# coop-columb/two-tower-amazon-recommender

Hardware: AMD Instinct MI355X
Metric: user-item pairs/sec (train step) + embedding-gather HBM GB/s, 1/2/4/8 MI355X (higher is better)
Workload: dtype f32; 1 GPU; cfg3: 5000000 users x 10000000 items, emb_dim 128, towers 128->256->128, batch 8192, in-batch sampled softmax T=0.1, sgd lr 1e-3, ids U; global_batch=8192, parallelism=single GPU

## Files before the change

### two_tower_amazon_recommender_amd/csrc/score.hip

```cpp
#include "common.h"

namespace {

using tt::f32x4;
using tt::f32x16;
typedef __bf16 bf16x4 __attribute__((ext_vector_type(4)));
typedef __bf16 bf16x8 __attribute__((ext_vector_type(8)));
typedef short s16x4 __attribute__((ext_vector_type(4)));

constexpr float kLog2e = 1.44269504088896340736f;
constexpr float kLn2 = 0.69314718055994530942f;
constexpr float kNegBig = -1.0e30f;

enum { MODE_FWD = 0, MODE_BWD = 1, MODE_FUSED = 2, MODE_RANK = 3, MODE_FUSED_S = 4, MODE_BWD_S = 5 };
constexpr float kRescaleThr = 8.0f;

struct ScoreArgs {
  const float* R;
  const float* K;
  int64_t n_r, n_c;
  int64_t diag;
  float c1;
  const float* a_r;
  const float* s_r;
  const float* a_c;
  const float* s_c;
  const int64_t* id_r;
  const int64_t* id_c;
  int nsplit;
  int64_t c_per_split;
  float* part_m;
  float* part_l;
  float* pos2;
  float* slab;
  const float* h_r;
  const float* h_c;
  const int64_t* pos_idx;
  int32_t* part_cnt;
  float* S;
  int64_t ldS;
};

template <int D, int PREC>
struct Geo {
  static constexpr int LS = D + 4;
  static constexpr int NG = D / 8;
  static constexpr int NB = D / 32;
  static constexpr int KS = D / 16;
  static constexpr int HALF_B = 32 * 256;
  static constexpr int PIECE_B = (D / 128) * HALF_B;
  static constexpr int TILE_F = PREC == 0 ? 32 * LS : 3 * PIECE_B / 4;
  static constexpr int BUF_F = TILE_F + 160;
  static constexpr int LDS_BYTES = 2 * BUF_F * 4;
};

struct Bf3 {
  __bf16 hi, mid, lo;
};
__device__ __forceinline__ Bf3 split3(float x) {
  Bf3 o;
  o.hi = (__bf16)x;
  const float r1 = x - (float)o.hi;
  o.mid = (__bf16)r1;
  o.lo = (__bf16)(r1 - (float)o.mid);
  return o;
}

__device__ __forceinline__ int img_off(int row, int ch) { return 256 * row + 16 * (ch ^ (((row & 3) << 2) | ((row >> 2) & 3))); }

constexpr int kBwdSWaves = 2;
constexpr int kSPrefetch = 2;
#ifndef TT_LOOP_LAMBDA
#define TT_LOOP_LAMBDA 0
#endif
constexpr int kTilesPerBarrier = 2;
constexpr int kTilesPerBarrierBwdS = kTilesPerBarrier;
template <int D, int MODE, int PREC>
constexpr int tiles_per_barrier() {
  if (PREC == 0 && D <= 128 && MODE == MODE_BWD_S) return kTilesPerBarrierBwdS;
  return (PREC == 0 && D <= 128 && (MODE == MODE_BWD || MODE == MODE_FUSED || MODE == MODE_FUSED_S))
             ? kTilesPerBarrier : 1;
}

template <int D, int MODE, int PREC>
constexpr bool split_d() {
  return PREC == 1 && D == 256 && (MODE == MODE_BWD || MODE == MODE_FUSED || MODE == MODE_FUSED_S);
}
template <int D, int MODE, bool HAS_IDS, bool HAS_HN, int PREC>
constexpr int rf_lds_groups() {
  if (PREC == 0 && D == 256 && (MODE == MODE_FUSED || MODE == MODE_FUSED_S) && (HAS_IDS || HAS_HN))
    return (HAS_IDS && HAS_HN) ? 10 : (HAS_HN ? 8 : 5);
  if (PREC == 0 && D == 128 && MODE == MODE_BWD && HAS_IDS && HAS_HN) return 2;
  return 0;
}
template <int D, int MODE, int PREC, int WAVES>
constexpr int rows_per_wg() { return (split_d<D, MODE, PREC>() ? WAVES / 2 : WAVES) * 32; }

template <int D, int MODE, bool HAS_IDS, bool HAS_HN, int WAVES, int PREC>
__global__ __launch_bounds__(WAVES * 64, (WAVES == 8 ? 2 : (D <= 128 ? ((MODE == MODE_BWD_S && PREC == 0) ? kBwdSWaves : 2) : 1))) void score_kernel(ScoreArgs p) {
  constexpr bool IS_FUSED = MODE == MODE_FUSED || MODE == MODE_FUSED_S;
  constexpr bool IS_BWD = MODE == MODE_BWD || MODE == MODE_BWD_S;
  constexpr bool FROM_S = MODE == MODE_BWD_S, TO_S = MODE == MODE_FUSED_S;
  using G_ = Geo<D, PREC>;
  constexpr int LS = G_::LS, NG = G_::NG, NB = G_::NB, TILE_F = G_::TILE_F, BUF_F = G_::BUF_F;
  constexpr int HALF_B = G_::HALF_B, PIECE_B = G_::PIECE_B;
  constexpr bool SPLIT = split_d<D, MODE, PREC>();
  constexpr int KS = SPLIT ? G_::KS / 2 : G_::KS;
  constexpr int NBW = SPLIT ? NB / 2 : NB;
  static_assert(PREC == 0 || D % 128 == 0, "bf16x3: dim 128 / 256 only (whole [32][128] bf16 images)");
  constexpr int ROW4 = D / 4;
  constexpr int THREADS = WAVES * 64;
  constexpr int NV = (32 * ROW4 + THREADS - 1) / THREADS;
  extern __shared__ __attribute__((aligned(16))) float smem[];

  const int tid = threadIdx.x;
  const int lane = tid & 63;
  const int wave = tid >> 6;
  const int h = lane >> 5;
  const int ln = lane & 31;

  const int split = __builtin_amdgcn_readfirstlane((int)(blockIdx.x % (unsigned)p.nsplit));
  const int64_t rblk = __builtin_amdgcn_readfirstlane((int)(blockIdx.x / (unsigned)p.nsplit));
  const int hw = SPLIT ? (wave & 1) : 0;
  const int64_t r0w = rblk * rows_per_wg<D, MODE, PREC, WAVES>() + (SPLIT ? wave >> 1 : wave) * 32;
  const int64_t r = r0w + ln;
  const bool r_ok = r < p.n_r;
  const int64_t c_begin = (int64_t)split * p.c_per_split;
  int64_t c_end = c_begin + p.c_per_split;
  if (c_end > p.n_c) c_end = p.n_c;
  const int ntiles = __builtin_amdgcn_readfirstlane(c_end > c_begin ? (int)((c_end - c_begin + 31) >> 5) : 0);

  constexpr bool RLO_LDS = PREC == 1 && WAVES == 8;
  constexpr int TPB = tiles_per_barrier<D, MODE, PREC>();
  static_assert(!(SPLIT && RLO_LDS), "wave-pair exchange buffer and the LDS lo fragments share one LDS region");
  static_assert(!SPLIT || TPB == 1, "the wave-pair exchange relies on one workgroup barrier per tile");
  constexpr int NBUF = 2 * TPB;
  constexpr int RFL = rf_lds_groups<D, MODE, HAS_IDS, HAS_HN, PREC>();
  constexpr int RFR = PREC == 0 ? NG - RFL : 1;
  f32x4 rf[RFR];
  f32x4* rfl = reinterpret_cast<f32x4*>(smem + NBUF * BUF_F) + (wave * (RFL > 0 ? RFL : 1)) * 64 + lane;
  bf16x8 rp[PREC == 0 ? 1 : (RLO_LDS ? 2 : 3)][PREC == 0 ? 1 : KS];
  bf16x8* rlo = reinterpret_cast<bf16x8*>(smem + NBUF * BUF_F) + (wave * KS) * 64 + lane;
  if constexpr (FROM_S) {
  } else if constexpr (PREC == 0) {
    const f32x4* R4 = reinterpret_cast<const f32x4*>(p.R + (r_ok ? r : 0) * D) + h;
#pragma unroll
    for (int g = 0; g < NG; ++g) {
      const f32x4 v = r_ok ? R4[2 * g] : f32x4{0.f, 0.f, 0.f, 0.f};
      if constexpr (RFL > 0) {
        if (g >= RFR) rfl[(g - RFR) * 64] = v; else rf[g < RFR ? g : 0] = v;
      } else {
        rf[g] = v;
      }
    }
  } else {
    const f32x4* R4 = reinterpret_cast<const f32x4*>(p.R + (r_ok ? r : 0) * D) + 2 * h + 32 * hw;
    const float live = r_ok ? 1.f : 0.f;
#pragma unroll
    for (int ks = 0; ks < KS; ++ks) {
      const f32x4 x0 = R4[4 * ks] * live;
      const f32x4 x1 = R4[4 * ks + 1] * live;
      bf16x8 lo8;
#pragma unroll
      for (int j = 0; j < 4; ++j) {
        const Bf3 u = split3(x0[j]), v = split3(x1[j]);
        rp[0][ks][j] = u.hi; rp[1][ks][j] = u.mid; lo8[j] = u.lo;
        rp[0][ks][4 + j] = v.hi; rp[1][ks][4 + j] = v.mid; lo8[4 + j] = v.lo;
      }
      if constexpr (RLO_LDS) rlo[ks * 64] = lo8;
      else rp[2][ks] = lo8;
    }
  }
  const float ar = ((IS_BWD || MODE == MODE_RANK) && p.a_r != nullptr && r_ok) ? p.a_r[r] : 0.f;
  const float sr = (IS_BWD && p.s_r != nullptr && r_ok) ? p.s_r[r] : 1.f;
  int64_t idr = 0;
  if constexpr (HAS_IDS) idr = r_ok ? p.id_r[r] : (int64_t)-1;
  const int64_t cpos = p.pos_idx != nullptr ? (r_ok ? p.pos_idx[r] : (int64_t)-1) : r + p.diag;

  f32x4 st[NV];
  float st_a = 0.f, st_s = 0.f, st_h = -3.0e38f;
  constexpr bool hn = HAS_HN;
  const float hr = (HAS_HN && p.h_r != nullptr && r_ok) ? p.h_r[r] : -3.0e38f;
  int64_t st_id = -2;
  constexpr int RPJ = THREADS / ROW4 > 0 ? THREADS / ROW4 : 1;
  const int st_row = tid / ROW4, st_col4 = tid % ROW4;
  const f32x4* kp = reinterpret_cast<const f32x4*>(p.K) + c_begin * ROW4;
  const bool has_ac = p.a_c != nullptr, has_sc = p.s_c != nullptr, has_hc = HAS_HN && p.h_c != nullptr;
  const float* acp = (has_ac ? p.a_c : p.K) + c_begin;
  const float* scp = (has_sc ? p.s_c : p.K) + c_begin;
  const float* hcp = (has_hc ? p.h_c : p.K) + c_begin;
  const int64_t* idp = nullptr;
  if constexpr (HAS_IDS) idp = p.id_c + c_begin;
  const int ncols = (int)(c_end - c_begin);

  auto load_tile = [&](int t) {
    const int nvalid = ncols - 32 * t;
    const int last = (nvalid < 32 ? nvalid : 32) - 1;
    const f32x4* src = kp + (int64_t)t * (32 * ROW4);
#pragma unroll
    for (int j = 0; j < NV; ++j) {
      const int row = st_row + j * RPJ;
      st[j] = src[(row < last ? row : last) * ROW4 + st_col4];
    }
    const int c = 32 * t + (tid < last ? tid : last);
    st_a = acp[c];
    if constexpr (HAS_HN) st_h = hcp[c];
    if constexpr (IS_BWD) st_s = scp[c];
    if constexpr (HAS_IDS) st_id = idp[c];
  };
  constexpr bool ST_FULL = NV * THREADS == 32 * ROW4;
  auto store_tile = [&](int t, int buf) {
    float* T = smem + buf * BUF_F;
    const int nvalid = ncols - 32 * t;
#pragma unroll
    for (int j = 0; j < NV; ++j) st[j] = (st_row + j * RPJ < nvalid) ? st[j] : f32x4{0.f, 0.f, 0.f, 0.f};
    if constexpr (!ST_FULL) {
#pragma unroll
      for (int j = 0; j < NV; ++j) asm volatile("" : : "v"(st[j]));
    }
    if constexpr (PREC == 0) {
      float* dst = T + st_row * LS + st_col4 * 4;
#pragma unroll
      for (int j = 0; j < NV; ++j)
        if (ST_FULL || st_row + j * RPJ < 32) *reinterpret_cast<f32x4*>(dst + j * RPJ * LS) = st[j];
    } else {
      char* img = reinterpret_cast<char*>(T);
      const int d0 = 4 * st_col4;
      const int sub = (d0 >> 7) * HALF_B + 8 * ((d0 >> 2) & 1), ch = (d0 & 127) >> 3;
#pragma unroll
      for (int j = 0; j < NV; ++j) {
        const int row = st_row + j * RPJ;
        if (ST_FULL || row < 32) {
          bf16x4 q0, q1, q2;
#pragma unroll
          for (int e = 0; e < 4; ++e) {
            const Bf3 u = split3(st[j][e]);
            q0[e] = u.hi; q1[e] = u.mid; q2[e] = u.lo;
          }
          char* dst = img + sub + img_off(row, ch);
          *reinterpret_cast<bf16x4*>(dst) = q0;
          *reinterpret_cast<bf16x4*>(dst + PIECE_B) = q1;
          *reinterpret_cast<bf16x4*>(dst + 2 * PIECE_B) = q2;
        }
      }
    }
    asm volatile("" : : "v"(st_a));
    if constexpr (IS_BWD) asm volatile("" : : "v"(st_s));
    if constexpr (HAS_HN) asm volatile("" : : "v"(st_h));
    if constexpr (HAS_IDS) asm volatile("" : : "v"(st_id));
    if (tid < 32) {
      const bool ok = tid < nvalid;
      T[TILE_F + tid] = ok ? (has_ac ? st_a : 0.f) : kNegBig;
      T[TILE_F + 32 + tid] = ok ? ((IS_BWD && has_sc) ? st_s : 1.f) : 0.f;
      if constexpr (HAS_HN) T[TILE_F + 128 + tid] = (ok && has_hc) ? st_h : -3.0e38f;
      if constexpr (HAS_IDS) reinterpret_cast<int64_t*>(T + TILE_F + 64)[tid] = ok ? st_id : (int64_t)-2;
    }
  };

  const bool frag_ok = __builtin_amdgcn_readfirstlane((int)(r0w < p.n_r)) != 0;
  auto store_S = [&](int t, const f32x16& X) {
    if (!frag_ok) return;
    const int64_t ctile = (c_begin >> 5) + t;
    float* blk = p.S + (ctile * p.ldS + (r0w >> 5)) * 1024 + ln * 32 + 4 * h;
#pragma unroll
    for (int g = 0; g < 4; ++g)
      if (!SPLIT || (g >> 1) == hw)
        *reinterpret_cast<f32x4*>(blk + 8 * g) = f32x4{X[4 * g], X[4 * g + 1], X[4 * g + 2], X[4 * g + 3]};
  };
  float* xch = smem + NBUF * BUF_F;
  auto exchange = [&](f32x16& X) {
    f32x4* mine = reinterpret_cast<f32x4*>(xch + wave * 1024) + lane;
    const f32x4* other = reinterpret_cast<const f32x4*>(xch + (wave ^ 1) * 1024) + lane;
#pragma unroll
    for (int g = 0; g < 4; ++g) mine[64 * g] = f32x4{X[4 * g], X[4 * g + 1], X[4 * g + 2], X[4 * g + 3]};
    __syncthreads();
#pragma unroll
    for (int g = 0; g < 4; ++g) {
      const f32x4 o = other[64 * g];
#pragma unroll
      for (int i = 0; i < 4; ++i) X[4 * g + i] += o[i];
    }
  };
  auto load_S = [&](int t, f32x16& X) {
    const int64_t q0 = c_begin + 32 * (int64_t)t;
    const float* blk = p.S + ((frag_ok ? (r0w >> 5) : 0) * p.ldS + (q0 >> 5)) * 1024 + 4 * h * 32 + ln;
#pragma unroll
    for (int reg = 0; reg < 16; ++reg) X[reg] = blk[tt::acc_row(reg, 0) * 32];
  };
  auto mask_S = [&](int t, const f32x16& Xin) -> f32x16 {
    const int nq_left = ncols - 32 * t;
    f32x16 X;
#pragma unroll
    for (int reg = 0; reg < 16; ++reg) X[reg] = (r_ok && (tt::acc_row(reg, 0) + 4 * h) < nq_left) ? Xin[reg] : 0.f;
    return X;
  };
  auto clamp_tile = [&](int t) { return t < ntiles ? t : ntiles - 1; };

  float run_m = kNegBig, run_l = 0.f, pos = 0.f;
  int cnt = 0;
  bool have_pos = false;
  f32x16 G[NBW];
  if constexpr (IS_BWD || IS_FUSED) {
#pragma unroll
    for (int b = 0; b < NBW; ++b)
#pragma unroll
      for (int i = 0; i < 16; ++i) G[b][i] = 0.f;
  }

#pragma unroll
  for (int t0 = 0; t0 < TPB; ++t0)
    if (t0 < ntiles) {
      load_tile(t0);
      store_tile(t0, t0);
    }
  __syncthreads();
  auto gemm1 = [&](const float* T) -> f32x16 {
    f32x16 X;
#pragma unroll
    for (int i = 0; i < 16; ++i) X[i] = 0.f;
    if constexpr (PREC == 1) {
      const char* img = reinterpret_cast<const char*>(T);
      auto frag = [&](int ks, bf16x8& f_hi, bf16x8& f_mid, bf16x8& f_lo, bf16x8& r_lo) {
        const int off = (SPLIT ? hw : (ks >> 3)) * HALF_B + img_off(ln, 2 * (ks & 7) + h);
        f_hi = *reinterpret_cast<const bf16x8*>(img + off);
        f_mid = *reinterpret_cast<const bf16x8*>(img + PIECE_B + off);
        f_lo = *reinterpret_cast<const bf16x8*>(img + 2 * PIECE_B + off);
        if constexpr (RLO_LDS) r_lo = rlo[ks * 64];
      };
      bf16x8 a_hi, a_mid, a_lo, b_lo = {};
      frag(0, a_hi, a_mid, a_lo, b_lo);
#pragma unroll
      for (int ks = 0; ks < KS; ++ks) {
        bf16x8 n_hi = a_hi, n_mid = a_mid, n_lo = a_lo, nb_lo = b_lo;
        if (ks + 1 < KS) frag(ks + 1, n_hi, n_mid, n_lo, nb_lo);
        if constexpr (!RLO_LDS) b_lo = rp[2][ks];
        X = __builtin_amdgcn_mfma_f32_32x32x16_bf16(a_lo, rp[0][ks], X, 0, 0, 0);
        X = __builtin_amdgcn_mfma_f32_32x32x16_bf16(a_hi, b_lo, X, 0, 0, 0);
        X = __builtin_amdgcn_mfma_f32_32x32x16_bf16(a_mid, rp[1][ks], X, 0, 0, 0);
        X = __builtin_amdgcn_mfma_f32_32x32x16_bf16(a_mid, rp[0][ks], X, 0, 0, 0);
        X = __builtin_amdgcn_mfma_f32_32x32x16_bf16(a_hi, rp[1][ks], X, 0, 0, 0);
        X = __builtin_amdgcn_mfma_f32_32x32x16_bf16(a_hi, rp[0][ks], X, 0, 0, 0);
        a_hi = n_hi; a_mid = n_mid; a_lo = n_lo; b_lo = nb_lo;
        __builtin_amdgcn_sched_barrier(0);
      }
    } else {
      const float* arow = T + ln * LS + 4 * h;
      f32x4 a_cur = *reinterpret_cast<const f32x4*>(arow);
#pragma unroll
      for (int g = 0; g < NG; ++g) {
        f32x4 a_nxt = a_cur;
        if (g + 1 < NG) a_nxt = *reinterpret_cast<const f32x4*>(arow + 8 * (g + 1));
        f32x4 rg;
        if constexpr (RFL > 0) { if (g >= RFR) rg = rfl[(g - RFR) * 64]; else rg = rf[g < RFR ? g : 0]; } else rg = rf[g];
        X = __builtin_amdgcn_mfma_f32_32x32x2f32(a_cur[0], rg[0], X, 0, 0, 0);
        X = __builtin_amdgcn_mfma_f32_32x32x2f32(a_cur[1], rg[1], X, 0, 0, 0);
        X = __builtin_amdgcn_mfma_f32_32x32x2f32(a_cur[2], rg[2], X, 0, 0, 0);
        X = __builtin_amdgcn_mfma_f32_32x32x2f32(a_cur[3], rg[3], X, 0, 0, 0);
        a_cur = a_nxt;
        __builtin_amdgcn_sched_barrier(0);
      }
    }
    return X;
  };

  auto epilogue = [&](const float* T, int t, const f32x16& X, float (&coef)[16]) {
    const int64_t c0 = c_begin + 32 * (int64_t)t;
    float ac[16], sc[16];
#pragma unroll
    for (int q = 0; q < 4; ++q) {
      const f32x4 va = *reinterpret_cast<const f32x4*>(T + TILE_F + 8 * q + 4 * h);
#pragma unroll
      for (int i = 0; i < 4; ++i) ac[4 * q + i] = va[i];
      if constexpr (IS_BWD) {
        const f32x4 vs = *reinterpret_cast<const f32x4*>(T + TILE_F + 32 + 8 * q + 4 * h);
#pragma unroll
        for (int i = 0; i < 4; ++i) sc[4 * q + i] = vs[i];
      }
    }
    float hth[16];
    if constexpr (hn) {
#pragma unroll
      for (int q = 0; q < 4; ++q) {
        const f32x4 vh = *reinterpret_cast<const f32x4*>(T + TILE_F + 128 + 8 * q + 4 * h);
#pragma unroll
        for (int i = 0; i < 4; ++i) hth[4 * q + i] = fmaxf(vh[i], hr);
      }
    }
    bool diag_tile;
    if (p.pos_idx != nullptr) {
      const int64_t dd0 = cpos - c0;
      diag_tile = __any(dd0 >= 0 && dd0 < 32) != 0;
    } else {
      diag_tile = (c0 < r0w + p.diag + 32) && (c0 + 32 > r0w + p.diag);
    }
    int dloc = -100;
    if (diag_tile) {
      const int64_t dd = cpos - c0;
      dloc = (dd >= 0 && dd < 32) ? (int)dd - 4 * h : -100;
    }
    auto take_pos = [&](bool hit, float v) {
      if constexpr (HAS_IDS) {
        if (hit) { pos = v; have_pos = true; }
      } else {
        pos = hit ? v : pos;
        have_pos = have_pos || hit;
      }
    };
    bool dup[16];
    if constexpr (HAS_IDS) {
      const int64_t* idc = reinterpret_cast<const int64_t*>(T + TILE_F + 64) + 4 * h;
#pragma unroll
      for (int reg = 0; reg < 16; ++reg)
        dup[reg] = (idc[tt::acc_row(reg, 0)] == idr) && (tt::acc_row(reg, 0) != dloc);
    }

    if constexpr (MODE == MODE_RANK) {
#pragma unroll
      for (int reg = 0; reg < 16; ++reg) {
        const float v = __builtin_fmaf(X[reg], p.c1, ac[reg]);
        bool above = v > ar && tt::acc_row(reg, 0) != dloc;
        if constexpr (HAS_IDS) above = above && !dup[reg];
        cnt += above ? 1 : 0;
      }
    } else if constexpr (MODE == MODE_FWD) {
      float t2[16];
      float mx = kNegBig;
#pragma unroll
      for (int reg = 0; reg < 16; ++reg) {
        float v = __builtin_fmaf(X[reg], p.c1, ac[reg]);
        if constexpr (HAS_IDS) v = dup[reg] ? kNegBig : v;
        if constexpr (hn) v = (v < hth[reg] && tt::acc_row(reg, 0) != dloc) ? kNegBig : v;
        t2[reg] = v;
        mx = fmaxf(mx, v);
      }
      if (diag_tile) {
#pragma unroll
        for (int reg = 0; reg < 16; ++reg) take_pos(tt::acc_row(reg, 0) == dloc, t2[reg]);
      }
      const float m_new = fmaxf(run_m, mx);
      float sum = 0.f;
#pragma unroll
      for (int reg = 0; reg < 16; ++reg) sum += __builtin_amdgcn_exp2f(t2[reg] - m_new);
      run_l = run_l * __builtin_amdgcn_exp2f(run_m - m_new) + sum;
      run_m = m_new;
    } else {
      if constexpr (IS_BWD) {
        float tvs[16];
#pragma unroll
        for (int reg = 0; reg < 16; ++reg) tvs[reg] = __builtin_fmaf(X[reg], p.c1, ac[reg]) + ar;
#pragma unroll
        for (int reg = 0; reg < 16; ++reg) {
          const float w = sc[reg] * sr;
          float tv = tvs[reg];
          if constexpr (hn) tv = (tv < hth[reg] && tt::acc_row(reg, 0) != dloc) ? kNegBig : tv;
          float e = __builtin_amdgcn_exp2f(tv) * w;
          if constexpr (HAS_IDS) e = dup[reg] ? 0.f : e;
          coef[reg] = e;
        }
        if (diag_tile) {
#pragma unroll
          for (int reg = 0; reg < 16; ++reg) {
            const float d = coef[reg] - sc[reg] * sr;
            coef[reg] = tt::acc_row(reg, 0) == dloc ? d : coef[reg];
          }
        }
      } else {
        float mx = kNegBig;
        float vs[16];
#pragma unroll
        for (int reg = 0; reg < 16; ++reg) vs[reg] = __builtin_fmaf(X[reg], p.c1, ac[reg]);
#pragma unroll
        for (int reg = 0; reg < 16; ++reg) {
          float v = vs[reg];
          if constexpr (HAS_IDS) v = dup[reg] ? kNegBig : v;
          if constexpr (hn) v = (v < hth[reg] && tt::acc_row(reg, 0) != dloc) ? kNegBig : v;
          coef[reg] = v;
          mx = fmaxf(mx, v);
        }
        if (diag_tile) {
#pragma unroll
          for (int reg = 0; reg < 16; ++reg) take_pos(tt::acc_row(reg, 0) == dloc, coef[reg]);
        }
        mx = fmaxf(mx, __shfl_xor(mx, 32));
        if (__any(mx - run_m > kRescaleThr)) {
          const float m_new = fmaxf(run_m, mx);
          const float alpha = __builtin_amdgcn_exp2f(run_m - m_new);
          run_l *= alpha;
#pragma unroll
          for (int b = 0; b < NBW; ++b)
#pragma unroll
            for (int i = 0; i < 16; ++i) G[b][i] *= alpha;
          run_m = m_new;
        }
        float s0 = 0.f, s1 = 0.f;
#pragma unroll
        for (int q = 0; q < 8; ++q) {
          coef[2 * q] = __builtin_amdgcn_exp2f(coef[2 * q] - run_m);
          coef[2 * q + 1] = __builtin_amdgcn_exp2f(coef[2 * q + 1] - run_m);
          s0 = q == 0 ? coef[0] : s0 + coef[2 * q];
          s1 = q == 0 ? coef[1] : s1 + coef[2 * q + 1];
        }
        run_l += s0 + s1;
      }
    }
  };

  auto gemm2 = [&](const float* T, const float (&coef)[16]) {
    if constexpr (PREC == 1) {
      bf16x8 c_hi[2], c_mid[2];
#pragma unroll
      for (int i = 0; i < 16; ++i) {
        const __bf16 hi = (__bf16)coef[i];
        c_hi[i >> 3][i & 7] = hi;
        c_mid[i >> 3][i & 7] = (__bf16)(coef[i] - (float)hi);
      }
      const char* img = reinterpret_cast<const char*>(T);
      const int g16 = (lane >> 4) & 1, q = (lane >> 2) & 3, pp = lane & 3;
      constexpr int NSTEP = 2 * NBW;
      auto frag = [&](int i, bf16x8& k_hi, bf16x8& k_mid) {
        const int b = i >> 1, s = i & 1;
        const int sub = (SPLIT ? hw : ((32 * b) >> 7)) * HALF_B + 8 * (pp & 1);
        const int ch = (((32 * b) & 127) >> 3) + 2 * g16 + (pp >> 1);
#pragma unroll
        for (int half = 0; half < 2; ++half) {
          const int row = 16 * s + 8 * half + 4 * h + q;
          const int off = sub + img_off(row, ch);
          const s16x4 v0 = __builtin_amdgcn_ds_read_tr16_b64_v4i16((__attribute__((address_space(3))) s16x4*)(img + off));
          const s16x4 v1 = __builtin_amdgcn_ds_read_tr16_b64_v4i16((__attribute__((address_space(3))) s16x4*)(img + PIECE_B + off));
#pragma unroll
          for (int e = 0; e < 4; ++e) {
            k_hi[4 * half + e] = __builtin_bit_cast(__bf16, (short)v0[e]);
            k_mid[4 * half + e] = __builtin_bit_cast(__bf16, (short)v1[e]);
          }
        }
      };
      bf16x8 k_hi, k_mid;
      frag(0, k_hi, k_mid);
#pragma unroll
      for (int i = 0; i < NSTEP; ++i) {
        bf16x8 n_hi = k_hi, n_mid = k_mid;
        if (i + 1 < NSTEP) frag(i + 1, n_hi, n_mid);
        const int b = i >> 1, s = i & 1;
        G[b] = __builtin_amdgcn_mfma_f32_32x32x16_bf16(k_mid, c_hi[s], G[b], 0, 0, 0);
        G[b] = __builtin_amdgcn_mfma_f32_32x32x16_bf16(k_hi, c_mid[s], G[b], 0, 0, 0);
        G[b] = __builtin_amdgcn_mfma_f32_32x32x16_bf16(k_hi, c_hi[s], G[b], 0, 0, 0);
        k_hi = n_hi; k_mid = n_mid;
        __builtin_amdgcn_sched_barrier(0);
      }
      return;
    } else {
      const float* kbase = T + 4 * h * LS + NB * ln;
      f32x4 kc0, kc1;
      auto read_k = [&](int reg, f32x4& k0, f32x4& k1) {
        const float* krow = kbase + tt::acc_row(reg, 0) * LS;
        if constexpr (NB == 8) {
          k0 = *reinterpret_cast<const f32x4*>(krow);
          k1 = *reinterpret_cast<const f32x4*>(krow + 4);
        } else if constexpr (NB == 4) {
          k0 = *reinterpret_cast<const f32x4*>(krow);
        } else if constexpr (NB == 2) {
          const float2 k2 = *reinterpret_cast<const float2*>(krow);
          k0[0] = k2.x; k0[1] = k2.y;
        } else {
          k0[0] = krow[0];
        }
      };
      read_k(0, kc0, kc1);
#pragma unroll
      for (int reg = 0; reg < 16; ++reg) {
        f32x4 kn0 = kc0, kn1 = kc1;
        if (reg + 1 < 16) read_k(reg + 1, kn0, kn1);
#pragma unroll
        for (int b = 0; b < (NB < 4 ? NB : 4); ++b)
          G[b] = __builtin_amdgcn_mfma_f32_32x32x2f32(kc0[b], coef[reg], G[b], 0, 0, 0);
        if constexpr (NB == 8) {
#pragma unroll
          for (int b = 0; b < 4; ++b)
            G[4 + b] = __builtin_amdgcn_mfma_f32_32x32x2f32(kc1[b], coef[reg], G[4 + b], 0, 0, 0);
        }
        kc0 = kn0; kc1 = kn1;
        __builtin_amdgcn_sched_barrier(0);
      }
    }
  };

  if constexpr (FROM_S && kSPrefetch == 2) {
    f32x16 xa, xb;
#pragma unroll
    for (int i = 0; i < 16; ++i) { xa[i] = 0.f; xb[i] = 0.f; }
    auto tile_step = [&](int t, f32x16& xs_t) {
      if constexpr (PREC == 1) load_tile(clamp_tile(t + 1));
      const float* T = smem + (t % NBUF) * BUF_F;
      const f32x16 X = mask_S(t, xs_t);
      float coef[16];
      epilogue(T, t, X, coef);
      if constexpr (PREC == 0) load_tile(clamp_tile(t + TPB));
      load_S(clamp_tile(t + 2), xs_t);
      gemm2(T, coef);
      store_tile(t + TPB, (t + TPB) % NBUF);
      if ((t % TPB) == TPB - 1) __syncthreads();
    };
    if (ntiles > 0) {
      load_S(0, xa);
      load_S(clamp_tile(1), xb);
      int t = 0;
      for (; t + 1 < ntiles; t += 2) {
        tile_step(t, xa);
        tile_step(t + 1, xb);
      }
      if (t < ntiles) tile_step(t, xa);
    }
  } else {
    f32x16 xs;
#pragma unroll
    for (int i = 0; i < 16; ++i) xs[i] = 0.f;
    if constexpr (FROM_S) { if (ntiles > 0) load_S(0, xs); }
#if TT_LOOP_LAMBDA
    auto tile_step = [&](int t) {
      if constexpr (MODE == MODE_FWD || MODE == MODE_RANK || PREC == 1) load_tile(clamp_tile(t + 1));
      const float* T = smem + (t % NBUF) * BUF_F;
      f32x16 X;
      if constexpr (FROM_S) X = mask_S(t, xs); else X = gemm1(T);
      if constexpr (SPLIT) exchange(X);
      if constexpr (TO_S) store_S(t, X);
      float coef[16];
      epilogue(T, t, X, coef);
      if constexpr (IS_BWD || IS_FUSED) {
        if constexpr (PREC == 0) load_tile(clamp_tile(t + TPB));
        if constexpr (FROM_S) load_S(clamp_tile(t + 1), xs);
        gemm2(T, coef);
      }
      store_tile(t + TPB, (t + TPB) % NBUF);
      if ((t % TPB) == TPB - 1) __syncthreads();
    };
    for (int t = 0; t < ntiles; t += 2) {
      tile_step(t);
      if (t + 1 < ntiles) tile_step(t + 1);
    }
#else
    for (int t = 0; t < ntiles; ++t) {
      if constexpr (MODE == MODE_FWD || MODE == MODE_RANK || PREC == 1) load_tile(clamp_tile(t + 1));
      const float* T = smem + (t % NBUF) * BUF_F;
      f32x16 X;
      if constexpr (FROM_S) X = mask_S(t, xs); else X = gemm1(T);
      if constexpr (SPLIT) exchange(X);
      if constexpr (TO_S) store_S(t, X);
      float coef[16];
      epilogue(T, t, X, coef);
      if constexpr (IS_BWD || IS_FUSED) {
        if constexpr (PREC == 0) load_tile(clamp_tile(t + TPB));
        if constexpr (FROM_S) load_S(clamp_tile(t + 1), xs);
        gemm2(T, coef);
      }
      store_tile(t + TPB, (t + TPB) % NBUF);
      if ((t % TPB) == TPB - 1) __syncthreads();
    }
#endif
  }

  if constexpr (IS_FUSED) {
    const float L = run_l + __shfl_xor(run_l, 32);
    if (r_ok && hw == 0) {
      if (h == 0) {
        p.part_m[(int64_t)split * p.n_r + r] = run_m;
        p.part_l[(int64_t)split * p.n_r + r] = L;
      }
      if (have_pos) p.pos2[r] = pos;
    }
  }
  if constexpr (MODE == MODE_RANK) {
    const int total = cnt + __shfl_xor(cnt, 32);
    if (r_ok && h == 0) p.part_cnt[(int64_t)split * p.n_r + r] = total;
  } else if constexpr (MODE == MODE_FWD) {
    const float om = __shfl_xor(run_m, 32);
    const float ol = __shfl_xor(run_l, 32);
    const float M = fmaxf(run_m, om);
    const float L = run_l * __builtin_amdgcn_exp2f(run_m - M) + ol * __builtin_amdgcn_exp2f(om - M);
    if (r_ok) {
      if (h == 0) {
        p.part_m[(int64_t)split * p.n_r + r] = M;
        p.part_l[(int64_t)split * p.n_r + r] = L;
      }
      if (have_pos) p.pos2[r] = pos;
    }
  } else {
    if (r_ok) {
      float* out = p.slab + ((int64_t)split * p.n_r + r) * D + 128 * hw;
      if constexpr (PREC == 1) {
#pragma unroll
        for (int b = 0; b < NBW; ++b)
#pragma unroll
          for (int g = 0; g < 4; ++g)
            *reinterpret_cast<f32x4*>(out + 32 * b + 8 * g + 4 * h) = f32x4{G[b][4 * g], G[b][4 * g + 1], G[b][4 * g + 2], G[b][4 * g + 3]};
      } else
#pragma unroll
      for (int reg = 0; reg < 16; ++reg) {
        const int i = tt::acc_row(reg, 0) + 4 * h;
        if constexpr (NB == 8) {
          *reinterpret_cast<f32x4*>(out + 8 * i) = f32x4{G[0][reg], G[1][reg], G[2][reg], G[3][reg]};
          *reinterpret_cast<f32x4*>(out + 8 * i + 4) = f32x4{G[4][reg], G[5][reg], G[6][reg], G[7][reg]};
        } else if constexpr (NB == 4) {
          *reinterpret_cast<f32x4*>(out + 4 * i) = f32x4{G[0][reg], G[1][reg], G[2][reg], G[3][reg]};
        } else if constexpr (NB == 2) {
          *reinterpret_cast<float2*>(out + 2 * i) = float2{G[0][reg], G[1][reg]};
        } else {
          out[i] = G[0][reg];
        }
      }
    }
  }
}


__global__ __launch_bounds__(256) void prob_bias_kernel(const float* __restrict__ prob, float* __restrict__ out, int64_t n) {
  const int64_t i = (int64_t)blockIdx.x * 256 + threadIdx.x;
  if (i < n) out[i] = -__log2f(fminf(fmaxf(prob[i], 1e-6f), 1.0f));
}

__global__ __launch_bounds__(256) void bwd_prep_kernel(const float* __restrict__ lse, const float* __restrict__ w,
                                                       float* __restrict__ a, float* __restrict__ s, int64_t n,
                                                       float scale) {
  const int64_t i = (int64_t)blockIdx.x * 256 + threadIdx.x;
  if (i < n) {
    a[i] = -lse[i] * kLog2e;
    s[i] = (w != nullptr ? w[i] : 1.0f) * scale;
  }
}

__global__ __launch_bounds__(256) void fwd_combine_kernel(const float* __restrict__ part_m, const float* __restrict__ part_l,
                                                          const float* __restrict__ pos2, const float* __restrict__ w,
                                                          int64_t n_r, int nsplit, float* __restrict__ lse,
                                                          float* __restrict__ per_row) {
  const int64_t r = (int64_t)blockIdx.x * 256 + threadIdx.x;
  if (r >= n_r) return;
  float M = kNegBig;
  for (int s = 0; s < nsplit; ++s) M = fmaxf(M, part_m[(int64_t)s * n_r + r]);
  float L = 0.f;
// ... 221 lines not shown
          if (r0 + 1024 * i + 256 * j < n_rows) a[j] += v[i][j];
    }
    red[t] = (a[0] + a[2]) + (a[1] + a[3]);
    __syncthreads();
    for (int s2 = 128; s2 > 0; s2 >>= 1) {
      if (t < s2) red[t] += red[t + s2];
      __syncthreads();
    }
    if (t == 0) loss[0] = red[0];
    return;
  }
  const int64_t nblk = per_row != nullptr ? gridDim.x - 1 : gridDim.x;
  const int64_t stride = nblk * 256;
  for (int64_t i = (int64_t)blockIdx.x * 256 + threadIdx.x; i < n4; i += stride) {
    f32x4 a = slab[i];
    for (int s = 1; s < nsplit; ++s) a += slab[(int64_t)s * n4 + i];
    out[i] = a;
  }
}


constexpr int kScoreWaves = 4;
constexpr int kScoreWgs = 512;
constexpr int kBwdSWgs = 512;
int choose_nsplit_pow2(int64_t n_r, int64_t n_c, int target_wgs = kScoreWgs) {
  const int64_t nrb = (n_r + 32 * kScoreWaves - 1) / (32 * kScoreWaves);
  int ns = 1;
  while (nrb * ns < target_wgs && (int64_t)ns * 2 * 64 <= n_c && ns < 64) ns *= 2;
  return ns;
}

int choose_nsplit(int64_t n_r, int64_t n_c, int rows_per_wg = 32 * kScoreWaves, int slots = kScoreWgs) {
  const int64_t nrb = (n_r + rows_per_wg - 1) / rows_per_wg;
  int best = 1;
  double best_cost = 0.0;
  for (int ns = 1; ns <= 64; ++ns) {
    if (ns > 1 && (int64_t)ns * 64 > n_c) break;
    const int64_t rounds = (nrb * ns + slots - 1) / slots;
    const double cost = (double)rounds / ns * (1.0 + 0.005 * ns);
    if (ns == 1 || cost < best_cost - 1e-12) { best = ns; best_cost = cost; }
  }
  return best;
}

int64_t align_up(int64_t x, int64_t a) { return (x + a - 1) / a * a; }

struct WsLayout {
  int ns_q, ns_c;
  int ns_cs;
  int64_t off_bias, off_aq, off_sq, off_hq, off_pm, off_pl, off_pos, off_slab, off_S, total_no_S, total;
};

WsLayout ws_layout(int64_t nq, int64_t nc, int32_t dim) {
  WsLayout w{};
  if (dim <= 128) {
    w.ns_q = choose_nsplit(nq, nc);
    w.ns_c = choose_nsplit(nc, nq);
    w.ns_cs = choose_nsplit(nc, nq, 256, 256);
  } else {
    w.ns_q = choose_nsplit_pow2(nq, nc);
    w.ns_c = choose_nsplit_pow2(nc, nq);
    w.ns_cs = choose_nsplit_pow2(nc, nq, kBwdSWgs);
  }
  int64_t o = 0;
  w.off_bias = o; o = align_up(o + nc * 4, 256);
  w.off_aq = o;   o = align_up(o + nq * 4, 256);
  w.off_sq = o;   o = align_up(o + nq * 4, 256);
  w.off_hq = o;   o = align_up(o + nq * 4, 256);
  w.off_pm = o;   o = align_up(o + (int64_t)w.ns_q * nq * 4, 256);
  w.off_pl = o;   o = align_up(o + (int64_t)w.ns_q * nq * 4, 256);
  w.off_pos = o;  o = align_up(o + nq * 4, 256);
  w.off_slab = o;
  const int64_t slab_q = (int64_t)w.ns_q * nq * dim * 4, slab_c = (int64_t)(w.ns_c > w.ns_cs ? w.ns_c : w.ns_cs) * nc * dim * 4;
  o = align_up(o + (slab_q > slab_c ? slab_q : slab_c), 256);
  w.total_no_S = o;
  w.off_S = o;
  o = align_up(o + ((nq + 31) / 32) * ((nc + 31) / 32) * 4096, 256);
  w.total = o;
  return w;
}

constexpr int kBwdSWgWaves = 8;
constexpr int kFusedSWgWaves = 4;
template <int D, int MODE, int PREC = 0>
constexpr int waves_for() {
  return (PREC == 1 && D == 128) ? 8 : (PREC == 1 ? 4 : ((MODE == MODE_BWD_S && D <= 128) ? kBwdSWgWaves
                                                         : ((MODE == MODE_FUSED_S && D <= 128) ? kFusedSWgWaves : kScoreWaves)));
}

template <int D, int MODE, int PREC = 0>
int launch_score(const ScoreArgs& a_in, bool has_ids, hipStream_t stream) {
  constexpr int W = waves_for<D, MODE, PREC>();
  constexpr int RPW = rows_per_wg<D, MODE, PREC, W>();
  const int64_t nrb = (a_in.n_r + RPW - 1) / RPW;
  const int64_t blocks = nrb * a_in.nsplit;
  const int lds_base = Geo<D, PREC>::LDS_BYTES * tiles_per_barrier<D, MODE, PREC>() +
                  ((PREC == 1 && W == 8) ? W * Geo<D, PREC>::KS * 64 * 16 : 0) +
                  (split_d<D, MODE, PREC>() ? W * 4096 : 0);
  const bool has_hn = (a_in.h_r != nullptr) || (a_in.h_c != nullptr);
  const ScoreArgs& a = a_in;
  auto go = [&](auto kern, int rfl_groups = 0) -> int {
    const int lds = lds_base + W * rfl_groups * 64 * 16;
    if (lds > 64 * 1024) {
      if (hipFuncSetAttribute(reinterpret_cast<const void*>(kern), hipFuncAttributeMaxDynamicSharedMemorySize, lds) != hipSuccess)
        return tt::fail(TT_ERR_LAUNCH, "hipFuncSetAttribute(LDS %d) failed", lds);
    }
    constexpr const char* tag = MODE == MODE_FWD ? "score_fwd" : ((MODE == MODE_BWD || MODE == MODE_BWD_S) ? "score_bwd"
                                : ((MODE == MODE_FUSED || MODE == MODE_FUSED_S) ? "score_fused" : "score_rank"));
    tt::launch(tag, kern, dim3((unsigned)blocks), dim3(W * 64), (unsigned)lds, stream, a);
    return tt::check_launch(tag);
  };
  if (has_ids && has_hn) return go(score_kernel<D, MODE, true, true, W, PREC>, rf_lds_groups<D, MODE, true, true, PREC>());
  if (has_ids) return go(score_kernel<D, MODE, true, false, W, PREC>, rf_lds_groups<D, MODE, true, false, PREC>());
  if (has_hn) return go(score_kernel<D, MODE, false, true, W, PREC>, rf_lds_groups<D, MODE, false, true, PREC>());
  return go(score_kernel<D, MODE, false, false, W, PREC>);
}

template <int MODE>
int dispatch_score_bx3(int32_t dim, const ScoreArgs& a, bool has_ids, hipStream_t stream) {
  switch (dim) {
    case 128: return launch_score<128, MODE, 1>(a, has_ids, stream);
    case 256: return launch_score<256, MODE, 1>(a, has_ids, stream);
    default: return tt::fail(TT_ERR_UNSUPPORTED, "retrieval (bf16x3): dim %d not in {128,256}", dim);
  }
}

template <int MODE>
int dispatch_score(int32_t dim, const ScoreArgs& a, bool has_ids, hipStream_t stream) {
  switch (dim) {
    case 32: return launch_score<32, MODE>(a, has_ids, stream);
    case 64: return launch_score<64, MODE>(a, has_ids, stream);
    case 128: return launch_score<128, MODE>(a, has_ids, stream);
    case 256: return launch_score<256, MODE>(a, has_ids, stream);
    default: return tt::fail(TT_ERR_UNSUPPORTED, "retrieval: dim %d not in {32,64,128,256}", dim);
  }
}

int check_common(const char* fn, const float* q, const float* c, int64_t nq, int64_t nc, int32_t dim,
                 int64_t diag_offset, const void* ws, int64_t ws_bytes, bool need_S = false) {
  TT_REQUIRE(q && c && ws, "%s: null pointer", fn);
  TT_REQUIRE(nq > 0 && nc > 0, "%s: nq and nc must be positive", fn);
  TT_REQUIRE(diag_offset >= 0 && nq + diag_offset <= nc, "%s: need 0 <= diag_offset and nq + diag_offset <= nc", fn);
  TT_REQUIRE(dim == 32 || dim == 64 || dim == 128 || dim == 256, "%s: dim %d not in {32,64,128,256}", fn, dim);
  TT_REQUIRE(tt::aligned16(q) && tt::aligned16(c), "%s: q/c must be 16-byte aligned", fn);
  TT_REQUIRE((reinterpret_cast<uintptr_t>(ws) & 255u) == 0, "%s: workspace must be 256-byte aligned", fn);
  const WsLayout wl = ws_layout(nq, nc, dim);
  const int64_t need = need_S ? wl.total : wl.total_no_S;
  if (ws_bytes < need)
    return tt::fail(TT_ERR_WORKSPACE, "%s: workspace %lld < %lld bytes", fn, (long long)ws_bytes, (long long)need);
  return TT_OK;
}

}

extern "C" int32_t tt_retrieval_num_splits(int64_t nq, int64_t nc, int32_t dim, int32_t pass) {
  if (nq <= 0 || nc <= 0 || dim <= 0 || pass < 0 || pass > 2) return 0;
  const WsLayout w = ws_layout(nq, nc, dim);
  return pass == 0 ? w.ns_q : (pass == 1 ? w.ns_c : w.ns_cs);
}

extern "C" int64_t tt_retrieval_workspace_bytes(int64_t nq, int64_t nc, int32_t dim) {
  if (nq <= 0 || nc <= 0 || dim <= 0) return 0;
  return ws_layout(nq, nc, dim).total;
}

extern "C" int64_t tt_retrieval_fwd_workspace_bytes(int64_t nq, int64_t nc, int32_t dim) {
  if (nq <= 0 || nc <= 0 || dim <= 0) return 0;
  return ws_layout(nq, nc, dim).total_no_S;
}

extern "C" int64_t tt_retrieval_rank_workspace_bytes(int64_t nq, int64_t nc, int32_t dim) {
  if (nq <= 0 || nc <= 0 || dim <= 0) return 0;
  return ws_layout(nq, nc, dim).off_pl;
}

static int retrieval_fwd(int prec, const float* q, const float* c, int64_t nq, int64_t nc, int32_t dim,
                         int64_t diag_offset, float inv_temperature, const float* sample_weight,
                         const float* cand_prob, const int64_t* cand_ids, const float* hard_thr,
                         void* workspace, int64_t workspace_bytes, float* lse, float* per_row, float* loss,
                         tt_stream_t stream_) {
  int rc = check_common("tt_retrieval_fwd_f32", q, c, nq, nc, dim, diag_offset, workspace, workspace_bytes);
  if (rc != TT_OK) return rc;
  TT_REQUIRE(lse && per_row && loss, "tt_retrieval_fwd_f32: null output pointer");
  hipStream_t stream = tt::as_stream(stream_);
  const WsLayout w = ws_layout(nq, nc, dim);
  char* ws = static_cast<char*>(workspace);
  float* bias = reinterpret_cast<float*>(ws + w.off_bias);
  if (cand_prob != nullptr) {
    hipLaunchKernelGGL(prob_bias_kernel, dim3((unsigned)((nc + 255) / 256)), dim3(256), 0, stream, cand_prob, bias, nc);
    if ((rc = tt::check_launch("prob_bias")) != TT_OK) return rc;
  }
  ScoreArgs a{};
  a.R = q; a.K = c; a.n_r = nq; a.n_c = nc; a.diag = diag_offset;
  a.c1 = kLog2e * inv_temperature;
// ... 329 lines not shown
```

Before: 15.00 million pairs/s.

## Add specialized fast score kernels for full tiles without column/row biases

Adds two template specializations of the score kernel (fused-to-S without column bias, backward-from-S without row terms). They are selected when there are no ids, no hard negatives, no pos_idx and the bias pointers are absent. Full tiles run in a separate main loop that skips bounds clamping, masking and the bias loads and LDS stores, and S reads and writes use unsigned offsets. This is meant to cut per-tile address arithmetic and memory traffic in the in-batch softmax score pass, at the cost of more template instantiations and code size.

```diff
diff --git a/two_tower_amazon_recommender_amd/csrc/score.hip b/two_tower_amazon_recommender_amd/csrc/score.hip
--- a/two_tower_amazon_recommender_amd/csrc/score.hip
+++ b/two_tower_amazon_recommender_amd/csrc/score.hip
@@ -12,7 +12,10 @@
 constexpr float kLn2 = 0.69314718055994530942f;
 constexpr float kNegBig = -1.0e30f;
 
-enum { MODE_FWD = 0, MODE_BWD = 1, MODE_FUSED = 2, MODE_RANK = 3, MODE_FUSED_S = 4, MODE_BWD_S = 5 };
+enum { MODE_FWD = 0, MODE_BWD = 1, MODE_FUSED = 2, MODE_RANK = 3, MODE_FUSED_S = 4, MODE_BWD_S = 5,
+       MODE_FUSED_S_NC = 6, MODE_BWD_S_NR = 7 };
+constexpr int base_mode(int m) { return m == MODE_FUSED_S_NC ? (int)MODE_FUSED_S : (m == MODE_BWD_S_NR ? (int)MODE_BWD_S : m); }
+template <bool B> struct BoolC { static constexpr bool value = B; };
 constexpr float kRescaleThr = 8.0f;
 
 struct ScoreArgs {
@@ -96,8 +99,15 @@
 template <int D, int MODE, int PREC, int WAVES>
 constexpr int rows_per_wg() { return (split_d<D, MODE, PREC>() ? WAVES / 2 : WAVES) * 32; }
 
-template <int D, int MODE, bool HAS_IDS, bool HAS_HN, int WAVES, int PREC>
-__global__ __launch_bounds__(WAVES * 64, (WAVES == 8 ? 2 : (D <= 128 ? ((MODE == MODE_BWD_S && PREC == 0) ? kBwdSWaves : 2) : 1))) void score_kernel(ScoreArgs p) {
+template <int D, int MODE_T, bool HAS_IDS, bool HAS_HN, int WAVES, int PREC>
+__global__ __launch_bounds__(WAVES * 64, (WAVES == 8 ? 2 : (D <= 128 ? ((base_mode(MODE_T) == MODE_BWD_S && PREC == 0) ? kBwdSWaves : 2) : 1))) void score_kernel(ScoreArgs p) {
+  constexpr int MODE = base_mode(MODE_T);
+  constexpr bool FAST = MODE_T != MODE;
+  static_assert(!FAST || (PREC == 0 && !HAS_IDS && !HAS_HN), "the fast forms: exact f32, no ids, no hard negatives");
+  constexpr BoolC<false> GEN{};
+  constexpr BoolC<true> FULL_TILE{};
+  constexpr bool NO_AC = FAST && MODE == MODE_FUSED_S;
+  constexpr bool NO_ROW = FAST && MODE == MODE_BWD_S;
   constexpr bool IS_FUSED = MODE == MODE_FUSED || MODE == MODE_FUSED_S;
   constexpr bool IS_BWD = MODE == MODE_BWD || MODE == MODE_BWD_S;
   constexpr bool FROM_S = MODE == MODE_BWD_S, TO_S = MODE == MODE_FUSED_S;
@@ -115,7 +125,7 @@
 
   const int tid = threadIdx.x;
   const int lane = tid & 63;
-  const int wave = tid >> 6;
+  const int wave = FAST ? __builtin_amdgcn_readfirstlane(tid >> 6) : tid >> 6;
   const int h = lane >> 5;
   const int ln = lane & 31;
 
@@ -129,6 +139,7 @@
   int64_t c_end = c_begin + p.c_per_split;
   if (c_end > p.n_c) c_end = p.n_c;
   const int ntiles = __builtin_amdgcn_readfirstlane(c_end > c_begin ? (int)((c_end - c_begin + 31) >> 5) : 0);
+  const int nfull = __builtin_amdgcn_readfirstlane(c_end > c_begin ? (int)((c_end - c_begin) >> 5) : 0);
 
   constexpr bool RLO_LDS = PREC == 1 && WAVES == 8;
   constexpr int TPB = tiles_per_barrier<D, MODE, PREC>();
@@ -171,8 +182,8 @@
       else rp[2][ks] = lo8;
     }
   }
-  const float ar = ((IS_BWD || MODE == MODE_RANK) && p.a_r != nullptr && r_ok) ? p.a_r[r] : 0.f;
-  const float sr = (IS_BWD && p.s_r != nullptr && r_ok) ? p.s_r[r] : 1.f;
+  const float ar = (!NO_ROW && (IS_BWD || MODE == MODE_RANK) && p.a_r != nullptr && r_ok) ? p.a_r[r] : 0.f;
+  const float sr = (!NO_ROW && IS_BWD && p.s_r != nullptr && r_ok) ? p.s_r[r] : 1.f;
   int64_t idr = 0;
   if constexpr (HAS_IDS) idr = r_ok ? p.id_r[r] : (int64_t)-1;
   const int64_t cpos = p.pos_idx != nullptr ? (r_ok ? p.pos_idx[r] : (int64_t)-1) : r + p.diag;
@@ -193,27 +204,41 @@
   if constexpr (HAS_IDS) idp = p.id_c + c_begin;
   const int ncols = (int)(c_end - c_begin);
 
-  auto load_tile = [&](int t) {
+  constexpr bool ST_FULL = NV * THREADS == 32 * ROW4;
+  auto load_tile = [&](int t, auto full) {
+    constexpr bool FULL = decltype(full)::value;
+    const f32x4* src = kp + (int64_t)t * (32 * ROW4);
+    if constexpr (FULL) {
+      static_assert(ST_FULL || NV == 1, "threads past row 31 exist only where a thread stages one float4");
+      const unsigned off0 = (unsigned)((ST_FULL ? st_row : (st_row < 31 ? st_row : 31)) * ROW4 + st_col4);
+#pragma unroll
+      for (int j = 0; j < NV; ++j) st[j] = (src + (ST_FULL ? j * RPJ * ROW4 : 0))[off0];
+      const unsigned c31 = (unsigned)(tid < 31 ? tid : 31);
+      if constexpr (!NO_AC) st_a = (acp + 32 * (int64_t)t)[c31];
+      if constexpr (IS_BWD) st_s = (scp + 32 * (int64_t)t)[c31];
+      return;
+    }
     const int nvalid = ncols - 32 * t;
     const int last = (nvalid < 32 ? nvalid : 32) - 1;
-    const f32x4* src = kp + (int64_t)t * (32 * ROW4);
 #pragma unroll
     for (int j = 0; j < NV; ++j) {
       const int row = st_row + j * RPJ;
       st[j] = src[(row < last ? row : last) * ROW4 + st_col4];
     }
     const int c = 32 * t + (tid < last ? tid : last);
-    st_a = acp[c];
+    if constexpr (!NO_AC) st_a = acp[c];
     if constexpr (HAS_HN) st_h = hcp[c];
     if constexpr (IS_BWD) st_s = scp[c];
     if constexpr (HAS_IDS) st_id = idp[c];
   };
-  constexpr bool ST_FULL = NV * THREADS == 32 * ROW4;
-  auto store_tile = [&](int t, int buf) {
+  auto store_tile = [&](int t, int buf, auto full) {
+    constexpr bool FULL = decltype(full)::value;
     float* T = smem + buf * BUF_F;
     const int nvalid = ncols - 32 * t;
-#pragma unroll
-    for (int j = 0; j < NV; ++j) st[j] = (st_row + j * RPJ < nvalid) ? st[j] : f32x4{0.f, 0.f, 0.f, 0.f};
+    if constexpr (!FULL) {
+#pragma unroll
+      for (int j = 0; j < NV; ++j) st[j] = (st_row + j * RPJ < nvalid) ? st[j] : f32x4{0.f, 0.f, 0.f, 0.f};
+    }
     if constexpr (!ST_FULL) {
 #pragma unroll
       for (int j = 0; j < NV; ++j) asm volatile("" : : "v"(st[j]));
@@ -243,6 +268,18 @@
           *reinterpret_cast<bf16x4*>(dst + 2 * PIECE_B) = q2;
         }
       }
+    }
+    if constexpr (NO_AC) {
+      return;
+    } else if constexpr (NO_ROW) {
+      asm volatile("" : : "v"(st_a));
+      asm volatile("" : : "v"(st_s));
+      if (tid < 32) {
+        const bool ok = FULL || tid < nvalid;
+        T[TILE_F + tid] = ok ? st_a : kNegBig;
+        T[TILE_F + 32 + tid] = ok ? st_s : 0.f;
+      }
+      return;
     }
     asm volatile("" : : "v"(st_a));
     if constexpr (IS_BWD) asm volatile("" : : "v"(st_s));
@@ -261,6 +298,13 @@
   auto store_S = [&](int t, const f32x16& X) {
     if (!frag_ok) return;
     const int64_t ctile = (c_begin >> 5) + t;
+    if constexpr (FAST) {
+      float* blk_u = p.S + (ctile * p.ldS + (r0w >> 5)) * 1024;
+      const unsigned lo = (unsigned)(ln * 32 + 4 * h);
+#pragma unroll
+      for (int g = 0; g < 4; ++g) *reinterpret_cast<f32x4*>(blk_u + (lo + 8u * g)) = f32x4{X[4 * g], X[4 * g + 1], X[4 * g + 2], X[4 * g + 3]};
+      return;
+    }
     float* blk = p.S + (ctile * p.ldS + (r0w >> 5)) * 1024 + ln * 32 + 4 * h;
 #pragma unroll
     for (int g = 0; g < 4; ++g)
@@ -283,6 +327,13 @@
   };
   auto load_S = [&](int t, f32x16& X) {
     const int64_t q0 = c_begin + 32 * (int64_t)t;
+    if constexpr (FAST) {
+      const float* blk_u = p.S + ((frag_ok ? (r0w >> 5) : 0) * p.ldS + (q0 >> 5)) * 1024;
+      const unsigned lo = (unsigned)(4 * h * 32 + ln);
+#pragma unroll
+      for (int reg = 0; reg < 16; ++reg) X[reg] = blk_u[lo + (unsigned)(tt::acc_row(reg, 0) * 32)];
+      return;
+    }
     const float* blk = p.S + ((frag_ok ? (r0w >> 5) : 0) * p.ldS + (q0 >> 5)) * 1024 + 4 * h * 32 + ln;
 #pragma unroll
     for (int reg = 0; reg < 16; ++reg) X[reg] = blk[tt::acc_row(reg, 0) * 32];
@@ -310,8 +361,8 @@
 #pragma unroll
   for (int t0 = 0; t0 < TPB; ++t0)
     if (t0 < ntiles) {
-      load_tile(t0);
-      store_tile(t0, t0);
+      load_tile(t0, GEN);
+      store_tile(t0, t0, GEN);
     }
   __syncthreads();
   auto gemm1 = [&](const float* T) -> f32x16 {
@@ -363,14 +414,18 @@
     return X;
   };
 
-  auto epilogue = [&](const float* T, int t, const f32x16& X, float (&coef)[16]) {
+  auto epilogue = [&](const float* T, int t, const f32x16& X, float (&coef)[16], auto full) {
+    constexpr bool FULL = decltype(full)::value;
     const int64_t c0 = c_begin + 32 * (int64_t)t;
     float ac[16], sc[16];
 #pragma unroll
     for (int q = 0; q < 4; ++q) {
-      const f32x4 va = *reinterpret_cast<const f32x4*>(T + TILE_F + 8 * q + 4 * h);
-#pragma unroll
-      for (int i = 0; i < 4; ++i) ac[4 * q + i] = va[i];
+      if constexpr (NO_AC) {
+      } else {
+        const f32x4 va = *reinterpret_cast<const f32x4*>(T + TILE_F + 8 * q + 4 * h);
+#pragma unroll
+        for (int i = 0; i < 4; ++i) ac[4 * q + i] = va[i];
+      }
       if constexpr (IS_BWD) {
         const f32x4 vs = *reinterpret_cast<const f32x4*>(T + TILE_F + 32 + 8 * q + 4 * h);
 #pragma unroll
@@ -447,10 +502,10 @@
       if constexpr (IS_BWD) {
         float tvs[16];
 #pragma unroll
-        for (int reg = 0; reg < 16; ++reg) tvs[reg] = __builtin_fmaf(X[reg], p.c1, ac[reg]) + ar;
+        for (int reg = 0; reg < 16; ++reg) tvs[reg] = NO_ROW ? __builtin_fmaf(X[reg], p.c1, ac[reg]) : __builtin_fmaf(X[reg], p.c1, ac[reg]) + ar;
 #pragma unroll
         for (int reg = 0; reg < 16; ++reg) {
-          const float w = sc[reg] * sr;
+          const float w = NO_ROW ? sc[reg] : sc[reg] * sr;
           float tv = tvs[reg];
           if constexpr (hn) tv = (tv < hth[reg] && tt::acc_row(reg, 0) != dloc) ? kNegBig : tv;
           float e = __builtin_amdgcn_exp2f(tv) * w;
@@ -460,7 +515,7 @@
         if (diag_tile) {
 #pragma unroll
           for (int reg = 0; reg < 16; ++reg) {
-            const float d = coef[reg] - sc[reg] * sr;
+            const float d = coef[reg] - (NO_ROW ? sc[reg] : sc[reg] * sr);
             coef[reg] = tt::acc_row(reg, 0) == dloc ? d : coef[reg];
           }
         }
@@ -468,7 +523,14 @@
         float mx = kNegBig;
         float vs[16];
 #pragma unroll
-        for (int reg = 0; reg < 16; ++reg) vs[reg] = __builtin_fmaf(X[reg], p.c1, ac[reg]);
+        for (int reg = 0; reg < 16; ++reg) {
+          if constexpr (NO_AC) {
+            const float v0 = X[reg] * p.c1;
+            vs[reg] = (FULL || tt::acc_row(reg, 0) + 4 * h < ncols - 32 * t) ? v0 : __builtin_fmaf(X[reg], p.c1, kNegBig);
+          } else {
+            vs[reg] = __builtin_fmaf(X[reg], p.c1, ac[reg]);
+          }
+        }
 #pragma unroll
         for (int reg = 0; reg < 16; ++reg) {
           float v = vs[reg];
@@ -589,21 +651,39 @@
 #pragma unroll
     for (int i = 0; i < 16; ++i) { xa[i] = 0.f; xb[i] = 0.f; }
     auto tile_step = [&](int t, f32x16& xs_t) {
-      if constexpr (PREC == 1) load_tile(clamp_tile(t + 1));
+      if constexpr (PREC == 1) load_tile(clamp_tile(t + 1), GEN);
       const float* T = smem + (t % NBUF) * BUF_F;
       const f32x16 X = mask_S(t, xs_t);
       float coef[16];
-      epilogue(T, t, X, coef);
-      if constexpr (PREC == 0) load_tile(clamp_tile(t + TPB));
+      epilogue(T, t, X, coef, GEN);
+      if constexpr (PREC == 0) load_tile(clamp_tile(t + TPB), GEN);
       load_S(clamp_tile(t + 2), xs_t);
       gemm2(T, coef);
-      store_tile(t + TPB, (t + TPB) % NBUF);
+      store_tile(t + TPB, (t + TPB) % NBUF, GEN);
+      if ((t % TPB) == TPB - 1) __syncthreads();
+    };
+    auto full_step = [&](int t, f32x16& xs_t) {
+      const float* T = smem + (t % NBUF) * BUF_F;
+      float coef[16];
+      epilogue(T, t, xs_t, coef, FULL_TILE);
+      load_tile(t + TPB, FULL_TILE);
+      load_S(t + 2, xs_t);
+      gemm2(T, coef);
+      store_tile(t + TPB, (t + TPB) % NBUF, FULL_TILE);
       if ((t % TPB) == TPB - 1) __syncthreads();
     };
     if (ntiles > 0) {
       load_S(0, xa);
       load_S(clamp_tile(1), xb);
       int t = 0;
+      if constexpr (FAST) {
+        static_assert(TPB <= 2, "full_step prefetches at most two tiles ahead");
+        const int nfast = (nfull > 2 ? nfull - 2 : 0) & ~1;
+        for (; t < nfast; t += 2) {
+          full_step(t, xa);
+          full_step(t + 1, xb);
+        }
+      }
       for (; t + 1 < ntiles; t += 2) {
         tile_step(t, xa);
         tile_step(t + 1, xb);
@@ -615,44 +695,61 @@
 #pragma unroll
     for (int i = 0; i < 16; ++i) xs[i] = 0.f;
     if constexpr (FROM_S) { if (ntiles > 0) load_S(0, xs); }
+    int t_first = 0;
+    if constexpr (FAST) {
+      static_assert(!FROM_S && !SPLIT, "the fast form of pass 1");
+      const int nfast = nfull > TPB ? nfull - TPB : 0;
+      for (int t = 0; t < nfast; ++t) {
+        const float* T = smem + (t % NBUF) * BUF_F;
+        const f32x16 X = gemm1(T);
+        store_S(t, X);
+        float coef[16];
+        epilogue(T, t, X, coef, FULL_TILE);
+        load_tile(t + TPB, FULL_TILE);
+        gemm2(T, coef);
+        store_tile(t + TPB, (t + TPB) % NBUF, FULL_TILE);
+        if ((t % TPB) == TPB - 1) __syncthreads();
+      }
+      t_first = nfast;
+    }
 #if TT_LOOP_LAMBDA
     auto tile_step = [&](int t) {
-      if constexpr (MODE == MODE_FWD || MODE == MODE_RANK || PREC == 1) load_tile(clamp_tile(t + 1));
+      if constexpr (MODE == MODE_FWD || MODE == MODE_RANK || PREC == 1) load_tile(clamp_tile(t + 1), GEN);
       const float* T = smem + (t % NBUF) * BUF_F;
       f32x16 X;
       if constexpr (FROM_S) X = mask_S(t, xs); else X = gemm1(T);
       if constexpr (SPLIT) exchange(X);
       if constexpr (TO_S) store_S(t, X);
       float coef[16];
-      epilogue(T, t, X, coef);
+      epilogue(T, t, X, coef, GEN);
       if constexpr (IS_BWD || IS_FUSED) {
-        if constexpr (PREC == 0) load_tile(clamp_tile(t + TPB));
+        if constexpr (PREC == 0) load_tile(clamp_tile(t + TPB), GEN);
         if constexpr (FROM_S) load_S(clamp_tile(t + 1), xs);
         gemm2(T, coef);
       }
-      store_tile(t + TPB, (t + TPB) % NBUF);
+      store_tile(t + TPB, (t + TPB) % NBUF, GEN);
       if ((t % TPB) == TPB - 1) __syncthreads();
     };
-    for (int t = 0; t < ntiles; t += 2) {
+    for (int t = t_first; t < ntiles; t += 2) {
       tile_step(t);
       if (t + 1 < ntiles) tile_step(t + 1);
     }
 #else
-    for (int t = 0; t < ntiles; ++t) {
-      if constexpr (MODE == MODE_FWD || MODE == MODE_RANK || PREC == 1) load_tile(clamp_tile(t + 1));
+    for (int t = t_first; t < ntiles; ++t) {
+      if constexpr (MODE == MODE_FWD || MODE == MODE_RANK || PREC == 1) load_tile(clamp_tile(t + 1), GEN);
       const float* T = smem + (t % NBUF) * BUF_F;
       f32x16 X;
       if constexpr (FROM_S) X = mask_S(t, xs); else X = gemm1(T);
       if constexpr (SPLIT) exchange(X);
       if constexpr (TO_S) store_S(t, X);
       float coef[16];
-      epilogue(T, t, X, coef);
+      epilogue(T, t, X, coef, GEN);
       if constexpr (IS_BWD || IS_FUSED) {
-        if constexpr (PREC == 0) load_tile(clamp_tile(t + TPB));
+        if constexpr (PREC == 0) load_tile(clamp_tile(t + TPB), GEN);
         if constexpr (FROM_S) load_S(clamp_tile(t + 1), xs);
         gemm2(T, coef);
       }
-      store_tile(t + TPB, (t + TPB) % NBUF);
+      store_tile(t + TPB, (t + TPB) % NBUF, GEN);
       if ((t % TPB) == TPB - 1) __syncthreads();
     }
 #endif
@@ -1040,8 +1137,9 @@
 
 constexpr int kBwdSWgWaves = 8;
 constexpr int kFusedSWgWaves = 4;
-template <int D, int MODE, int PREC = 0>
+template <int D, int MODE_T, int PREC = 0>
 constexpr int waves_for() {
+  constexpr int MODE = base_mode(MODE_T);
   return (PREC == 1 && D == 128) ? 8 : (PREC == 1 ? 4 : ((MODE == MODE_BWD_S && D <= 128) ? kBwdSWgWaves
                                                          : ((MODE == MODE_FUSED_S && D <= 128) ? kFusedSWgWaves : kScoreWaves)));
 }
@@ -1068,6 +1166,18 @@
     tt::launch(tag, kern, dim3((unsigned)blocks), dim3(W * 64), (unsigned)lds, stream, a);
     return tt::check_launch(tag);
   };
+  if constexpr (PREC == 0 && (MODE == MODE_FUSED_S || MODE == MODE_BWD_S)) {
+    if (!has_ids && !has_hn && a.pos_idx == nullptr) {
+      if constexpr (MODE == MODE_FUSED_S) {
+        if constexpr (D == 64 || D == 128) {
+          if (a.a_c == nullptr) return go(score_kernel<D, MODE_FUSED_S_NC, false, false, W, 0>);
+        }
+      } else {
+        if (a.a_r == nullptr && a.s_r == nullptr && a.a_c != nullptr && a.s_c != nullptr)
+          return go(score_kernel<D, MODE_BWD_S_NR, false, false, W, 0>);
+      }
+    }
+  }
   if (has_ids && has_hn) return go(score_kernel<D, MODE, true, true, W, PREC>, rf_lds_groups<D, MODE, true, true, PREC>());
   if (has_ids) return go(score_kernel<D, MODE, true, false, W, PREC>, rf_lds_groups<D, MODE, true, false, PREC>());
   if (has_hn) return go(score_kernel<D, MODE, false, true, W, PREC>, rf_lds_groups<D, MODE, false, true, PREC>());
```

After: 15.44 million pairs/s (median of 6 runs). 1.03x the previous value.
